# MathisWellmann/gym-rs

Measured on AMD Instinct MI355X. Metric: env-steps/sec (whole node), CartPole-v1 @ 2^20 envs per MI355X, higher is better.
Workload: dtype f32

## Files before the change

### gym-rs_amd/csrc/gymrs_philox.h

```cpp
#pragma once
#include "gymrs_math.h"

namespace gymrs {

struct u32x4 {
    uint32_t v[4];
};

constexpr uint32_t kPhiloxM0 = 0xD2511F53u, kPhiloxM1 = 0xCD9E8D57u;
constexpr uint32_t kPhiloxW0 = 0x9E3779B9u, kPhiloxW1 = 0xBB67AE85u;

GYMRS_HD uint32_t xor3(uint32_t a, uint32_t b, uint32_t c)
{
#if defined(__HIP_DEVICE_COMPILE__)
    return __builtin_amdgcn_bitop3_b32(a, b, c, 0x96);
#else
    return a ^ b ^ c;
#endif
}

GYMRS_HD u32x4 philox4x32_10(uint32_t c0, uint32_t c1, uint32_t c2, uint32_t c3, uint32_t k0, uint32_t k1)
{
#if defined(__HIPCC__)
#pragma unroll
#endif
    for (int round = 0; round < 10; ++round) {
        uint64_t p0 = (uint64_t)kPhiloxM0 * c0;
        uint64_t p1 = (uint64_t)kPhiloxM1 * c2;
        uint32_t n0 = xor3((uint32_t)(p1 >> 32), c1, k0);
        uint32_t n2 = xor3((uint32_t)(p0 >> 32), c3, k1);
        c1 = (uint32_t)p1;
        c3 = (uint32_t)p0;
        c0 = n0;
        c2 = n2;
        k0 += kPhiloxW0;
        k1 += kPhiloxW1;
    }
    return u32x4{{c0, c1, c2, c3}};
}

constexpr uint32_t kStreamReset = 0, kStreamAction = 1;

GYMRS_HD u32x4 draw4(uint64_t seed, uint64_t gid, uint64_t tick, uint32_t stream)
{
    return philox4x32_10((uint32_t)gid, (uint32_t)(gid >> 32), (uint32_t)tick,
                         ((uint32_t)(tick >> 32) & 0xffffu) | (stream << 16), (uint32_t)seed,
                         (uint32_t)(seed >> 32));
}

GYMRS_HD u32x4 action_block(uint64_t seed, uint64_t gid, uint64_t slot) { return draw4(seed, gid >> 2, slot, kStreamAction); }
GYMRS_HD uint32_t pick_word(const u32x4& b, uint32_t j) { return j == 0 ? b.v[0] : (j == 1 ? b.v[1] : (j == 2 ? b.v[2] : b.v[3])); }
GYMRS_HD uint32_t action_word(uint64_t seed, uint64_t gid, uint64_t t) { return pick_word(action_block(seed, gid, t), (uint32_t)gid & 3u); }
GYMRS_HD uint8_t discrete_from_word(uint32_t word, uint64_t t, uint32_t n_actions)
{
    const uint32_t half = (word >> (((uint32_t)t & 1u) * 16u)) & 0xffffu;
    return (uint8_t)((half * n_actions) >> 16);
}
GYMRS_HD uint8_t action_discrete(uint64_t seed, uint64_t gid, uint64_t t, uint32_t n_actions)
{
    return discrete_from_word(action_word(seed, gid, t >> 1), t, n_actions);
}

struct SampleBox {
    float lo[4], scale24[4], hi_prev[4];
};

inline SampleBox make_sample_box(const float* lo, const float* hi, int dims)
{
    SampleBox b;
    for (int j = 0; j < 4; ++j) {
        b.lo[j] = 0.0f;
        b.scale24[j] = 0.0f;
        b.hi_prev[j] = 0.0f;
    }
    for (int j = 0; j < dims; ++j) {
        b.lo[j] = lo[j];
        b.scale24[j] = (hi[j] - lo[j]) * 0x1p-24f;
        uint32_t h = f2u(hi[j]);
        h = (hi[j] > 0.0f) ? h - 1u : ((h & 0x7fffffffu) == 0u ? 0x80000001u : h + 1u);
        b.hi_prev[j] = u2f(h);
    }
    return b;
}

GYMRS_HD float uniform_in_box(uint32_t r, const SampleBox& b, int j)
{
    const float v = fmaf_((float)(r >> 8), b.scale24[j], b.lo[j]);
    return v < b.hi_prev[j] ? v : b.hi_prev[j];
}

GYMRS_HD float uniform_between(uint32_t r, float low, float high)
{
    SampleBox b;
    b.lo[0] = low;
    b.scale24[0] = (high - low) * 0x1p-24f;
    uint32_t h = f2u(high);
    h = (high > 0.0f) ? h - 1u : ((h & 0x7fffffffu) == 0u ? 0x80000001u : h + 1u);
    b.hi_prev[0] = u2f(h);
    return uniform_in_box(r, b, 0);
}

}
```

### gym-rs_amd/csrc/gymrs_step_impl.h

```cpp
#pragma once
#include "gymrs_tile.h"

namespace gymrs {

__device__ __forceinline__ uint32_t select_by_mask(unsigned long long m, uint32_t fresh, uint32_t ep)
{
    uint32_t r;
    asm("v_cndmask_b32_e64 %0, %1, %2, %3" : "=v"(r) : "v"(ep), "v"(fresh), "s"(m));
    return r;
}

template <class Env, int VEC, uint32_t FLAGS, int THREADS, bool FULL>
__device__ __forceinline__ void step_block_loaded(StepArgs a, const typename Env::Consts& c, ResetLds<Env, VEC, THREADS>& lds, uint32_t vblock,
                                                  TileRegs<Env, VEC, FLAGS>& d)
{
    constexpr int kVec = VEC;
    constexpr int LPB = THREADS * kVec;
    constexpr bool AUTO = (FLAGS & GYMRS_AUTO_RESET) != 0;
    constexpr bool STATS = AUTO && (FLAGS & GYMRS_TRACK_STATS);
    constexpr bool LOGGED = TileRegs<Env, VEC, FLAGS>::LOGGED;
    const uint64_t base = (uint64_t)vblock * LPB + (uint64_t)threadIdx.x * kVec;
    if (a.tick_base) a.tick += *a.tick_base;
    unsigned long long old_resets = 0;
    double old_ret = 0.0, open = 0.0;
    const size_t wave_slot = (size_t)vblock * (THREADS / 64) + (threadIdx.x >> 6);
    if (STATS && !LOGGED) {
        const unsigned long long* bs = a.block_stats + wave_slot * 2;
        old_resets = bs[0];
        if (!Env::kConstReward) {
            old_ret = reinterpret_cast<const double*>(bs)[1];
            open = a.wave_open[wave_slot];
        }
    }
    constexpr int kOlder = (int)kResetLogRows - 1;
    Vec<uint32_t, VEC> ep;
    unsigned long long older = 0;
    [[maybe_unused]] unsigned long long* older_at = nullptr;
    const bool fold = LOGGED && a.fold_step != 0;
    if (fold) {
        ep = load_vec<uint32_t, kVec, false>(a.ep_start, base, a.n, FULL, 0u);
        const uint32_t lane = threadIdx.x & 63u;
        older_at = a.reset_log + (size_t)((uint32_t)(a.tick - 1 - (uint64_t)(lane / kVec)) & (kResetLogRows - 1u)) * a.reset_log_row_words +
                   wave_slot * kVec + lane % kVec;
        if (lane < (uint32_t)(kOlder * kVec)) older = *older_at;
        old_resets = a.block_stats[wave_slot * 2];
    }
    constexpr bool CAN_ELIDE = AUTO && Env::kConstReward;
    const bool elide = CAN_ELIDE && (Env::kElideConstReward || a.elide_reward != 0u);
    uint32_t clean = 0;
    if (elide) clean = a.wave_clean[wave_slot];
#ifndef GYMRS_EXP_XCC_PARTS
#define GYMRS_EXP_XCC_PARTS 7
#endif
    uint32_t xcc_want = 0, xcc_id = 0;
    const bool xcc_asks = a.xcc_check != 0u && (uint32_t)__builtin_amdgcn_readfirstlane((int)threadIdx.x) < 64u && vblock == blockIdx.x * (uint32_t)kStepTiles;
#if GYMRS_EXP_XCC_PARTS & 1
    if (xcc_asks && a.xcc_check == 1u) xcc_want = a.xcc_table[(blockIdx.x & 7u) * kXccTableStride];
#endif
#if GYMRS_EXP_XCC_PARTS & 2
    if (xcc_asks) {
        asm volatile("s_getreg_b32 %0, hwreg(HW_REG_XCC_ID)" : "=s"(xcc_id));
        xcc_id = (a.xcc_seq << 8) | ((xcc_id & 0xfu) + 1u);
    }
#endif
    GYMRS_STAMP(1);
    StepOut<VEC> out;
    advance_tile<Env, VEC, FLAGS, FULL, false, THREADS>(a, c, base, d, lds, old_resets, old_ret, open, out, vblock);
    store_tile<Env, VEC, FLAGS, FULL>(a, base, d, out, elide && clean != 0 && out.reward_is_const);
    if (fold) {
        const uint32_t lane = threadIdx.x & 63u;
        uint32_t finished = wave_sum_u32((uint32_t)__popcll(older));
#pragma unroll
        for (int k = 0; k < kVec; ++k) finished += (uint32_t)__popcll(out.masks[k]);
        if (finished != 0) {
#pragma unroll
            for (int s = kOlder - 1; s >= 0; --s) {
                const uint32_t fresh = (uint32_t)(a.tick - (uint64_t)s);
#pragma unroll
                for (int k = 0; k < kVec; ++k) {
                    const unsigned long long m = ((unsigned long long)(uint32_t)__builtin_amdgcn_readlane((int)(uint32_t)(older >> 32), s * kVec + k) << 32) |
                                                 (uint32_t)__builtin_amdgcn_readlane((int)(uint32_t)older, s * kVec + k);
                    ep.v[k] = select_by_mask(m, fresh, ep.v[k]);
                }
            }
            const uint32_t fresh_now = (uint32_t)(a.tick + 1);
#pragma unroll
            for (int k = 0; k < kVec; ++k) ep.v[k] = select_by_mask(out.masks[k], fresh_now, ep.v[k]);
            store_vec<uint32_t, kVec, false>(a.ep_start, base, a.n, FULL, ep);
            if (older != 0) *older_at = 0;
            if (lane == 0) a.block_stats[wave_slot * 2] = old_resets + finished;
        }
    }
    if (elide && (clean != 0) != out.reward_is_const && (threadIdx.x & 63u) == 0) a.wave_clean[wave_slot] = out.reward_is_const ? 1u : 0u;
    if (STATS && !Env::kConstReward && (threadIdx.x & 63u) == 0) a.wave_open[wave_slot] = open;
#if GYMRS_EXP_XCC_PARTS & 4
    if (xcc_asks) {
        if (a.xcc_check == 2u) {
            if (blockIdx.x < 8u && threadIdx.x == 0) a.xcc_table[blockIdx.x * kXccTableStride] = xcc_id;
        } else if (xcc_want != xcc_id && threadIdx.x == 0) {
            a.err_seen[1] = blockIdx.x + 1u;
        }
    }
#endif
    GYMRS_STAMP(6);
}

template <class Env, int VEC, uint32_t FLAGS, int THREADS, bool FULL>
__device__ __forceinline__ void step_block(const StepArgs& a, const typename Env::Consts& c, ResetLds<Env, VEC, THREADS>& lds, uint32_t vblock)
{
    GYMRS_STAMP(0);
    TileRegs<Env, VEC, FLAGS> d;
    load_tile<Env, VEC, FLAGS, FULL>(a, (uint64_t)vblock * (THREADS * VEC) + (uint64_t)threadIdx.x * VEC, d);
    load_param_index<Env, VEC, FLAGS, FULL>(a, c, (uint64_t)vblock * (THREADS * VEC) + (uint64_t)threadIdx.x * VEC, d);
    step_block_loaded<Env, VEC, FLAGS, THREADS, FULL>(a, c, lds, vblock, d);
}

template <class Env>
struct KernArgView {
    using Consts = typename Env::Consts;
    static __device__ __forceinline__ void fetch(StepArgs& a, Consts& c)
    {
        const char* kp = (const char*)__builtin_amdgcn_kernarg_segment_ptr();
        __builtin_memcpy(&a, kp + offsetof(StepKernArgs<Consts>, rest), sizeof(StepArgs));
        __builtin_memcpy(&c, kp + offsetof(StepKernArgs<Consts>, c), sizeof(Consts));
    }
};

template <class Env, int VEC, uint32_t FLAGS, int THREADS>
__device__ __forceinline__ void step_kernel_body(float* s0, float* s1, float* s2, float* s3, const void* action, uint64_t n_fast, const StepArgs& rest,
                                                 const typename Env::Consts& c_by_value)
{
    constexpr int LPB = THREADS * VEC;
    __shared__ ResetLds<Env, VEC, THREADS> lds;
    if constexpr (kStepTiles == 1 && Env::kLoadsAheadOfArguments) {
        StepArgs a;
        typename Env::Consts c;
        if ((uint64_t)blockIdx.x * LPB + (uint64_t)((threadIdx.x >> 6) + 1) * (64 * VEC) <= n_fast) {
#ifdef GYMRS_TRACE_TIMES
            const unsigned long long t_start = __builtin_amdgcn_s_memtime();
#endif
            using R = TileRegs<Env, VEC, FLAGS>;
            using Action = typename Env::Action;
            const uint64_t base = (uint64_t)blockIdx.x * LPB + (uint64_t)threadIdx.x * VEC;
            float* const sp[4] = {s0, s1, s2, s3};
            TileRegs<Env, VEC, FLAGS> d;
#pragma unroll
            for (int j = 0; j < Env::kState; ++j) d.st[j] = load_vec<float, VEC, R::NT_SL>(sp[j], base, n_fast, true, 0.0f);
            d.act = load_vec<Action, VEC, R::NT_A>(static_cast<const Action*>(action), base, n_fast, true, Action(0));
            __builtin_amdgcn_sched_barrier(0);
            KernArgView<Env>::fetch(a, c);
            a.s[0] = s0;
            a.s[1] = s1;
            a.s[2] = s2;
            a.s[3] = s3;
            a.action = action;
#ifdef GYMRS_TRACE_TIMES
            if (a.trace && (threadIdx.x & 63u) == 0) a.trace[((size_t)blockIdx.x * a.trace_wpb + (threadIdx.x >> 6)) * 8 + 0] = t_start;
#endif
            if (Env::kHasBeyond && !R::AUTO) d.beyond = load_vec<uint8_t, VEC, R::NT_SL>(a.beyond, base, a.n, true, uint8_t(0));
            if (R::TLIM && !Env::kNeverTerminates) d.ep_start = load_vec<uint32_t, VEC, false>(a.ep_start, base, a.n, true, 0u);
            load_param_index<Env, VEC, FLAGS, true>(a, c, base, d);
            step_block_loaded<Env, VEC, FLAGS, THREADS, true>(a, c, lds, blockIdx.x, d);
        } else {
            KernArgView<Env>::fetch(a, c);
            a.s[0] = s0;
            a.s[1] = s1;
            a.s[2] = s2;
            a.s[3] = s3;
            a.action = action;
            step_block<Env, VEC, FLAGS, THREADS, false>(a, c, lds, blockIdx.x);
        }
    } else {
        const typename Env::Consts& c = c_by_value;
        StepArgs a = rest;
        a.s[0] = s0;
        a.s[1] = s1;
        a.s[2] = s2;
        a.s[3] = s3;
        a.action = action;
        if constexpr (kStepTiles == 1) {
            if ((uint64_t)blockIdx.x * LPB + (uint64_t)((threadIdx.x >> 6) + 1) * (64 * VEC) <= n_fast)
                step_block<Env, VEC, FLAGS, THREADS, true>(a, c, lds, blockIdx.x);
            else
                step_block<Env, VEC, FLAGS, THREADS, false>(a, c, lds, blockIdx.x);
        } else {
            const uint32_t vb0 = blockIdx.x * (uint32_t)kStepTiles;
            if ((uint64_t)(vb0 + kStepTiles - 1) * LPB + (uint64_t)((threadIdx.x >> 6) + 1) * (64 * VEC) <= n_fast) {
                TileRegs<Env, VEC, FLAGS> d[2];
                load_tile<Env, VEC, FLAGS, true>(a, (uint64_t)vb0 * LPB + (uint64_t)threadIdx.x * VEC, d[0]);
                load_param_index<Env, VEC, FLAGS, true>(a, c, (uint64_t)vb0 * LPB + (uint64_t)threadIdx.x * VEC, d[0]);
#pragma unroll
                for (int j = 0; j < kStepTiles; ++j) {
                    if (j + 1 < kStepTiles) {
                        load_tile<Env, VEC, FLAGS, true>(a, (uint64_t)(vb0 + j + 1) * LPB + (uint64_t)threadIdx.x * VEC, d[(j + 1) & 1]);
                        load_param_index<Env, VEC, FLAGS, true>(a, c, (uint64_t)(vb0 + j + 1) * LPB + (uint64_t)threadIdx.x * VEC, d[(j + 1) & 1]);
                    }
                    step_block_loaded<Env, VEC, FLAGS, THREADS, true>(a, c, lds, vb0 + j, d[j & 1]);
                }
            } else {
                for (int j = 0; j < kStepTiles; ++j)
                    if ((uint64_t)(vb0 + j) * LPB < rest.n) step_block<Env, VEC, FLAGS, THREADS, false>(a, c, lds, vb0 + j);
            }
        }
    }
}

#ifndef GYMRS_EXP_WAVES
#define GYMRS_EXP_WAVES(VEC_) (16 / (VEC_) < 1 ? 1 : 16 / (VEC_))
#endif
#ifndef GYMRS_EXP_WAVES_MIN
#define GYMRS_EXP_WAVES_MIN 1
#endif
#define GYMRS_STEP_KERNEL_ATTRS(THREADS_, VEC_) \
    __global__ __launch_bounds__(THREADS_) __attribute__((amdgpu_waves_per_eu(GYMRS_EXP_WAVES_MIN, GYMRS_EXP_WAVES(VEC_))))

template <class Env, int VEC, uint32_t FLAGS, int THREADS>
GYMRS_STEP_KERNEL_ATTRS(THREADS, VEC) void step_kernel(float* s0, float* s1, float* s2, float* s3, const void* action, uint64_t n_fast,
                                                       const StepArgs rest, const typename Env::Consts c)
{
    step_kernel_body<Env, VEC, FLAGS, THREADS>(s0, s1, s2, s3, action, n_fast, rest, c);
}

#ifndef GYMRS_EXP_BLOCK
static_assert(CartPoleT::kThreads == kCartPoleThreads && MountainCarT::kThreads == kBlock && PendulumT::kThreads == kBlock,
              "step_threads_of (gymrs_kernels.h) must pick what launch_one picks");
#endif

template <class Env, int VEC, uint32_t FLAGS>
static hipError_t launch_one(const StepArgs& a, const void* consts, hipStream_t stream)
{
    launch_begin();
    if constexpr (Env::kThreads != kBlock) {
        if (step_uses_big_groups(a.n, Env::kThreads, VEC)) {
            hipLaunchKernelGGL((step_kernel<Env, VEC, FLAGS, Env::kThreads>), dim3(step_grid(a.n, VEC, Env::kThreads * kStepTiles)), dim3(Env::kThreads), 0,
                               stream, a.s[0], a.s[1], a.s[2], a.s[3], a.action, a.n_fast, a, *static_cast<const typename Env::Consts*>(consts));
            return hipGetLastError();
        }
    }
    hipLaunchKernelGGL((step_kernel<Env, VEC, FLAGS, kBlock>), dim3(step_grid(a.n, VEC, kBlock * kStepTiles)), dim3(kBlock), 0, stream, a.s[0], a.s[1],
                       a.s[2], a.s[3], a.action, a.n_fast, a, *static_cast<const typename Env::Consts*>(consts));
    return hipGetLastError();
}

template <class Env, int VEC, uint32_t NTBIT>
static hipError_t launch_flags_nt(uint32_t flags, const StepArgs& a, const void* consts, hipStream_t stream)
{
    constexpr uint32_t A = GYMRS_AUTO_RESET, S = GYMRS_TRACK_STATS, T = GYMRS_TIME_LIMIT, F = GYMRS_FINAL_OBS;
    if (!(flags & A)) flags &= ~(S | F);
    switch (flags & (A | S | T | F)) {
#ifdef GYMRS_DEV_MINIMAL
    case A | S: return launch_one<Env, VEC, A | S | NTBIT>(a, consts, stream);
    case A | S | T: return launch_one<Env, VEC, A | S | T | NTBIT>(a, consts, stream);
    default: return hipErrorInvalidValue;
#else
    case 0: return launch_one<Env, VEC, 0 | NTBIT>(a, consts, stream);
    case A: return launch_one<Env, VEC, A | NTBIT>(a, consts, stream);
    case A | S: return launch_one<Env, VEC, A | S | NTBIT>(a, consts, stream);
    case T: return launch_one<Env, VEC, T | NTBIT>(a, consts, stream);
    case A | T: return launch_one<Env, VEC, A | T | NTBIT>(a, consts, stream);
    case A | S | T: return launch_one<Env, VEC, A | S | T | NTBIT>(a, consts, stream);
    case A | F: return launch_one<Env, VEC, A | F | NTBIT>(a, consts, stream);
    case A | S | F: return launch_one<Env, VEC, A | S | F | NTBIT>(a, consts, stream);
    case A | T | F: return launch_one<Env, VEC, A | T | F | NTBIT>(a, consts, stream);
    case A | S | T | F: return launch_one<Env, VEC, A | S | T | F | NTBIT>(a, consts, stream);
    default: return hipErrorInvalidValue;
#endif
    }
}

template <class Env, int VEC>
static hipError_t launch_flags(uint32_t flags, const StepArgs& a, const void* consts, hipStream_t stream)
{
    if (flags & kFlagNonTemporal) return launch_flags_nt<Env, VEC, kFlagNonTemporal>(flags, a, consts, stream);
    if (flags & kFlagNtOut) return launch_flags_nt<Env, VEC, kFlagNtOut>(flags, a, consts, stream);
    return launch_flags_nt<Env, VEC, 0u>(flags, a, consts, stream);
}

template <class Env>
static hipError_t launch_vec(int vec, uint32_t flags, const StepArgs& a, const void* consts, hipStream_t stream)
{
    switch (vec) {
    case 4: return launch_flags<Env, 4>(flags, a, consts, stream);
#ifndef GYMRS_DEV_MINIMAL
    case 8: return launch_flags<Env, 8>(flags, a, consts, stream);
#endif
    default: return hipErrorInvalidValue;
    }
}

}
```

### gym-rs_amd/csrc/gymrs_tile.h

```cpp
#pragma once
#include <type_traits>

#include "gymrs_kernels.h"

namespace gymrs {


#ifdef GYMRS_TRACE_TIMES
#define GYMRS_STAMP(slot_)                                                                                   \
    do {                                                                                                     \
        if (a.trace && (threadIdx.x & 63u) == 0)                                                             \
            a.trace[((size_t)blockIdx.x * a.trace_wpb + (threadIdx.x >> 6)) * 8 + (slot_)] = __builtin_amdgcn_s_memtime(); \
    } while (0)
#else
#define GYMRS_STAMP(slot_) do { } while (0)
#endif

__device__ __forceinline__ float wave_sum(float v)
{
    auto dpp_add = [](float x, auto ctrl, auto row_mask) {
        const int moved = __builtin_amdgcn_update_dpp(0, __builtin_bit_cast(int, x), decltype(ctrl)::value, decltype(row_mask)::value, 0xf, true);
        return x + __builtin_bit_cast(float, moved);
    };
    using std::integral_constant;
    v = dpp_add(v, integral_constant<int, 0xb1>{}, integral_constant<int, 0xf>{});
    v = dpp_add(v, integral_constant<int, 0x4e>{}, integral_constant<int, 0xf>{});
    v = dpp_add(v, integral_constant<int, 0x141>{}, integral_constant<int, 0xf>{});
    v = dpp_add(v, integral_constant<int, 0x140>{}, integral_constant<int, 0xf>{});
    v = dpp_add(v, integral_constant<int, 0x142>{}, integral_constant<int, 0xa>{});
    v = dpp_add(v, integral_constant<int, 0x143>{}, integral_constant<int, 0xc>{});
    return __builtin_bit_cast(float, __builtin_amdgcn_readlane(__builtin_bit_cast(int, v), 63));
}

__device__ __forceinline__ uint32_t wave_sum_u32(uint32_t v)
{
    auto dpp_add = [](uint32_t x, auto ctrl, auto row_mask) {
        return x + (uint32_t)__builtin_amdgcn_update_dpp(0, (int)x, decltype(ctrl)::value, decltype(row_mask)::value, 0xf, true);
    };
    using std::integral_constant;
    v = dpp_add(v, integral_constant<int, 0xb1>{}, integral_constant<int, 0xf>{});
    v = dpp_add(v, integral_constant<int, 0x4e>{}, integral_constant<int, 0xf>{});
    v = dpp_add(v, integral_constant<int, 0x141>{}, integral_constant<int, 0xf>{});
    v = dpp_add(v, integral_constant<int, 0x140>{}, integral_constant<int, 0xf>{});
    v = dpp_add(v, integral_constant<int, 0x142>{}, integral_constant<int, 0xa>{});
    v = dpp_add(v, integral_constant<int, 0x143>{}, integral_constant<int, 0xc>{});
    return (uint32_t)__builtin_amdgcn_readlane((int)v, 63);
}

template <class T, int V>
struct alignas(sizeof(T) * V) Vec {
    T v[V];
};

template <class T, int V, bool NT>
__device__ __forceinline__ Vec<T, V> load_vec(const T* __restrict__ p, uint64_t base, uint64_t n, bool full, T fill)
{
    typedef T vt __attribute__((ext_vector_type(V)));
    Vec<T, V> r;
    if (full) {
        const vt x = NT ? __builtin_nontemporal_load(reinterpret_cast<const vt*>(p + base)) : *reinterpret_cast<const vt*>(p + base);
#pragma unroll
        for (int k = 0; k < V; ++k) r.v[k] = x[k];
    } else {
#pragma unroll
        for (int k = 0; k < V; ++k) r.v[k] = (base + k < n) ? p[base + k] : fill;
    }
    return r;
}

template <class T, int V, int POL>
__device__ __forceinline__ void store_vec(T* __restrict__ p, uint64_t base, uint64_t n, bool full, const Vec<T, V>& r)
{
    typedef T vt __attribute__((ext_vector_type(V)));
    if (full) {
        vt x;
#pragma unroll
        for (int k = 0; k < V; ++k) x[k] = r.v[k];
        if constexpr (POL == 2) {
            static_assert(sizeof(vt) == 4 || sizeof(vt) == 16, "sc1 stores: 4 lanes per work-item only");
            if constexpr (sizeof(vt) == 16) {
                typedef uint32_t u4 __attribute__((ext_vector_type(4)));
                asm volatile("global_store_dwordx4 %0, %1, off sc1\n\ts_nop 1" ::"v"(reinterpret_cast<vt*>(p + base)), "v"(__builtin_bit_cast(u4, x)) : "memory");
            }
            else
                asm volatile("global_store_dword %0, %1, off sc1\n\ts_nop 1" ::"v"(reinterpret_cast<vt*>(p + base)), "v"(__builtin_bit_cast(uint32_t, x)) : "memory");
        } else if constexpr (POL == 1)
            __builtin_nontemporal_store(x, reinterpret_cast<vt*>(p + base));
        else
            *reinterpret_cast<vt*>(p + base) = x;
    } else {
#pragma unroll
        for (int k = 0; k < V; ++k)
            if (base + k < n) p[base + k] = r.v[k];
    }
}

template <int VEC>
__device__ __forceinline__ void obs_sincos(const Vec<float, VEC>& theta, Vec<float, VEC>& oc, Vec<float, VEC>& os)
{
    bool med = true;
#pragma unroll
    for (int k = 0; k < VEC; ++k) med = med && in_short_range(theta.v[k]);
    if (__all(med)) {
#pragma unroll
        for (int k = 0; k < VEC; ++k) sincos_short(theta.v[k], &os.v[k], &oc.v[k]);
    } else {
#pragma unroll
        for (int k = 0; k < VEC; ++k) sincosf_(theta.v[k], &os.v[k], &oc.v[k]);
    }
}

struct CartPoleT {
    using Consts = CartPoleConsts;
    static constexpr bool kTable = false;
    using Action = uint8_t;
    static constexpr int kState = 4;
    static constexpr int kSampled = 4;
    static constexpr bool kConstReward = true;
    static constexpr float kReward = 1.0f;
    static constexpr bool kElideConstReward = false;
#ifdef GYMRS_EXP_NO_RESET_LOG
    static constexpr bool kUseResetLog = false;
#else
    static constexpr bool kUseResetLog = true;
#endif
    static constexpr bool kHasBeyond = true;
    static constexpr bool kHasObsExtra = false;
    static constexpr bool kNeverTerminates = false;
    static constexpr int kThreads = 512;
    static constexpr bool kLoadsAheadOfArguments = true;
    __device__ static bool valid(Action a) { return a < 2; }
    __device__ static void advance(const Consts& c, float* st, Action a, float& reward, bool& done)
    {
        done = cartpole_advance(c, st[0], st[1], st[2], st[3], a);
        reward = 1.0f;
    }
    static constexpr uint32_t kActions = 2;
    static constexpr uint32_t kRangeMax = 0x3f490fdbu;
    __device__ static uint32_t range_key(const float* st) { return f2u(st[2]) & 0x7fffffffu; }
    static constexpr int kVariants = 2;
    __device__ static int variant(const Consts& c) { return c.integrator == 0 ? 0 : 1; }
    template <int INTEG>
    __device__ static void advance_fast(const Consts& c, float* st, Action a, float& reward, bool& done)
    {
        done = cartpole_advance<SinCosSmall, INTEG>(c, st[0], st[1], st[2], st[3], a);
        reward = 1.0f;
    }
    __device__ static void sample(const u32x4& r, const SampleBox& b, float* st) { cartpole_sample(r, b, st[0], st[1], st[2], st[3]); }
};

struct MountainCarT {
    using Consts = MountainCarConsts;
    static constexpr bool kTable = false;
    using Action = uint8_t;
    static constexpr int kState = 2;
    static constexpr int kSampled = 1;
    static constexpr bool kConstReward = true;
    static constexpr float kReward = -1.0f;
    static constexpr bool kElideConstReward = true;
    static constexpr bool kUseResetLog = false;
    static constexpr bool kHasBeyond = false;
    static constexpr bool kHasObsExtra = false;
    static constexpr bool kNeverTerminates = false;
    static constexpr int kThreads = 256;
    static constexpr bool kLoadsAheadOfArguments = false;
    __device__ static bool valid(Action a) { return a < 3; }
    __device__ static void advance(const Consts& c, float* st, Action a, float& reward, bool& done)
    {
        done = mountain_car_advance(c, st[0], st[1], a);
        reward = -1.0f;
    }
    static constexpr uint32_t kActions = 3;
    static constexpr uint32_t kRangeMax = 0x43480000u;
    __device__ static uint32_t range_key(const float* st) { return f2u(3.0f * st[0]) & 0x7fffffffu; }
    static constexpr int kVariants = 1;
    __device__ static int variant(const Consts&) { return 0; }
    template <int>
    __device__ static void advance_fast(const Consts& c, float* st, Action a, float& reward, bool& done)
    {
        done = mountain_car_advance<SinCosShort>(c, st[0], st[1], a);
        reward = -1.0f;
    }
    __device__ static void sample(const u32x4& r, const SampleBox& b, float* st) { mountain_car_sample(r, b, st[0], st[1]); }
};

struct PendulumT {
    using Consts = PendulumConsts;
    static constexpr bool kTable = false;
    using Action = float;
    static constexpr int kState = 2;
    static constexpr int kSampled = 2;
    static constexpr bool kConstReward = false;
    static constexpr float kReward = 0.0f;
    static constexpr bool kElideConstReward = false;
    static constexpr bool kUseResetLog = false;
    static constexpr bool kHasBeyond = false;
    static constexpr bool kHasObsExtra = true;
    static constexpr bool kNeverTerminates = true;
    static constexpr int kThreads = 256;
    static constexpr bool kLoadsAheadOfArguments = true;
    __device__ static bool valid(Action) { return true; }
    __device__ static void advance(const Consts& c, float* st, Action a, float& reward, bool& done)
    {
        reward = pendulum_advance(c, st[0], st[1], a);
        done = false;
    }
    static constexpr uint32_t kActions = 0;
    static constexpr uint32_t kRangeMax = 0x43480000u;
    __device__ static uint32_t range_key(const float* st) { return f2u(st[0]) & 0x7fffffffu; }
    static constexpr int kVariants = 1;
    __device__ static int variant(const Consts&) { return 0; }
    template <int>
    __device__ static void advance_fast(const Consts& c, float* st, Action a, float& reward, bool& done)
    {
        reward = pendulum_advance<SinCosShort>(c, st[0], st[1], a);
        done = false;
    }
    __device__ static void sample(const u32x4& r, const SampleBox& b, float* st) { pendulum_sample(r, b, st[0], st[1]); }
};

template <class Base>
struct TableT : Base {
    static_assert(!Base::kNeverTerminates, "no Pendulum tables: max_torque also drives the random-policy actions");
    static constexpr bool kTable = true;
    using LaneConsts = typename Base::Consts;
    using Consts = TableConsts;
    __device__ static int variant(const Consts& c) { return Base::kVariants == 1 || c.integrator == 0 ? 0 : 1; }
    __device__ static LaneConsts lane_consts(const Consts& c, const ParamRow& r)
    {
        LaneConsts l;
        consts_of_row(r, c.integrator, c.max_steps, l);
        return l;
    }
};

template <class Env, class = void>
struct TableLane {
    struct type {};
};
template <class Env>
struct TableLane<Env, std::enable_if_t<Env::kTable>> {
    using type = typename Env::LaneConsts;
};

template <class Env, int VEC, uint32_t FLAGS>
struct TileRegs {
    static constexpr bool AUTO = (FLAGS & GYMRS_AUTO_RESET) != 0;
    static constexpr bool STATS = AUTO && (FLAGS & GYMRS_TRACK_STATS) != 0;
    static constexpr bool TLIM = (FLAGS & GYMRS_TIME_LIMIT) != 0;
    static constexpr bool FINAL = AUTO && (FLAGS & GYMRS_FINAL_OBS) != 0;
    static_assert(!FINAL || !(Env::kHasBeyond && !AUTO), "StepArgs::final_obs shares the slot of `beyond`: no FINAL kernel may read beyond");
    static constexpr bool NT = (FLAGS & kFlagNonTemporal) != 0;
#ifdef GYMRS_EXP_HINTS
    static constexpr bool NT_SL = (GYMRS_EXP_HINTS & 1) != 0, NT_SS = (GYMRS_EXP_HINTS & 2) != 0, NT_A = (GYMRS_EXP_HINTS & 4) != 0,
                          NT_O = (GYMRS_EXP_HINTS & 8) != 0;
#else
    static constexpr bool NT_SL = NT || (FLAGS & kFlagNtStateLoads) != 0, NT_SS = NT, NT_A = NT, NT_O = NT || (FLAGS & kFlagNtOut) != 0;
#endif
#ifdef GYMRS_EXP_SC1
    static constexpr int POL_SS = (VEC == 4 && (GYMRS_EXP_SC1 & 2)) ? 2 : (NT_SS ? 1 : 0), POL_O = (VEC == 4 && (GYMRS_EXP_SC1 & 8)) ? 2 : (NT_O ? 1 : 0);
#else
    static constexpr int POL_SS = NT_SS ? 1 : 0, POL_O = NT_O ? 1 : 0;
#endif
    static constexpr bool LOGGED = STATS && !TLIM && Env::kConstReward && Env::kUseResetLog;
    Vec<float, VEC> st[Env::kState];
    Vec<typename Env::Action, VEC> act;
    Vec<uint8_t, VEC> beyond;
    Vec<uint32_t, VEC> ep_start;
    Vec<uint16_t, VEC> pidx;
};

template <class Env, int VEC, uint32_t FLAGS, bool FULL>
__device__ __forceinline__ void load_param_index(const StepArgs& a, const typename Env::Consts& c, uint64_t base, TileRegs<Env, VEC, FLAGS>& d)
{
    if constexpr (Env::kTable) d.pidx = load_vec<uint16_t, VEC, false>(c.index, base, a.n, FULL, uint16_t(0));
}

template <class Env, int VEC, uint32_t FLAGS, bool FULL, bool ROLL = false>
__device__ __forceinline__ void load_tile(const StepArgs& a, uint64_t base, TileRegs<Env, VEC, FLAGS>& d)
{
    constexpr int kVec = VEC;
    using R = TileRegs<Env, VEC, FLAGS>;
    using Action = typename Env::Action;
#pragma unroll
    for (int j = 0; j < Env::kState; ++j) d.st[j] = load_vec<float, kVec, R::NT_SL>(a.s[j], base, a.n, FULL, 0.0f);
    if (!ROLL) d.act = load_vec<Action, kVec, R::NT_A>(static_cast<const Action*>(a.action), base, a.n, FULL, Action(0));
    if (Env::kHasBeyond && !R::AUTO) d.beyond = load_vec<uint8_t, kVec, R::NT_SL>(a.beyond, base, a.n, FULL, uint8_t(0));
    if (ROLL ? (R::STATS || R::TLIM) : (R::TLIM && !Env::kNeverTerminates))
        d.ep_start = load_vec<uint32_t, kVec, false>(a.ep_start, base, a.n, FULL, 0u);
}

template <class Env, int VEC, int THREADS = Env::kThreads>
struct ResetLds {
    static constexpr int kLanes = THREADS * VEC;
    uint16_t list[kLanes];
    struct alignas(Env::kState * 4) State {
        float v[Env::kState];
    };
    State fresh[kLanes];
};

template <class Env, int VEC, int V>
__device__ __forceinline__ void advance_fast_all(const typename Env::Consts& c, float (&ls)[Env::kState][VEC],
                                                 const typename Env::Action (&la)[VEC], float (&rw)[VEC], bool (&dn)[VEC])
{
    constexpr int kVec = VEC;
    constexpr int NS = Env::kState;
#pragma unroll
    for (int k = 0; k < kVec; ++k) {
        float lane_st[NS];
#pragma unroll
        for (int j = 0; j < NS; ++j) lane_st[j] = ls[j][k];
        Env::template advance_fast<V>(c, lane_st, la[k], rw[k], dn[k]);
#pragma unroll
        for (int j = 0; j < NS; ++j) ls[j][k] = lane_st[j];
    }
}

template <class Env, int VEC, int V>
__device__ __forceinline__ void advance_fast_rows(const typename Env::LaneConsts (&lc)[VEC], float (&ls)[Env::kState][VEC],
                                                  const typename Env::Action (&la)[VEC], float (&rw)[VEC], bool (&dn)[VEC])
{
    constexpr int NS = Env::kState;
#pragma unroll
    for (int k = 0; k < VEC; ++k) {
        float lane_st[NS];
#pragma unroll
        for (int j = 0; j < NS; ++j) lane_st[j] = ls[j][k];
        Env::template advance_fast<V>(lc[k], lane_st, la[k], rw[k], dn[k]);
#pragma unroll
        for (int j = 0; j < NS; ++j) ls[j][k] = lane_st[j];
    }
}

template <class Env, int VEC, uint32_t FLAGS>
__device__ __forceinline__ bool lane_index_ok(const typename Env::Consts& c, const TileRegs<Env, VEC, FLAGS>& d, int k)
{
    if constexpr (Env::kTable)
        return d.pidx.v[k] < c.k;
    else
        return true;
}

template <uint32_t N, class A, int VEC>
__device__ __forceinline__ bool actions_all_below(const Vec<A, VEC>& act)
{
    if constexpr (N == 0 || sizeof(A) != 1) {
        return true;
    } else {
        static_assert(N == 2 || N == 3, "only Discrete(2) and Discrete(3) are packed here");
        struct Words {
            uint32_t w[VEC / 4];
        };
        const Words words = __builtin_bit_cast(Words, act);
        uint32_t bad = 0;
#pragma unroll
        for (int i = 0; i < VEC / 4; ++i) {
            const uint32_t x = words.w[i];
            bad |= N == 2 ? (x & 0xfefefefeu) : ((x & 0xfcfcfcfcu) | (x & (x >> 1) & 0x01010101u));
        }
        return bad == 0;
    }
}

template <int VEC>
struct StepOut {
    Vec<float, VEC> reward;
    Vec<uint8_t, VEC> done, trunc;
    bool reward_is_const;
    unsigned long long masks[VEC];
};

template <class Env, int VEC, uint32_t FLAGS, bool FULL>
__device__ __forceinline__ void store_final_obs(const StepArgs& a, uint64_t base, const float (&ls)[Env::kState][VEC], const bool (&need_reset)[VEC])
{
    using R = TileRegs<Env, VEC, FLAGS>;
    static_assert(R::FINAL, "final-observation stores belong to GYMRS_FINAL_OBS instantiations only");
    const uint64_t stride = final_obs_stride(a.n);
    float* const fo = a.final_obs;
    if constexpr (Env::kHasObsExtra) {
        static_assert(Env::kNeverTerminates && Env::kState == 2, "the obs_extra env is Pendulum: (cos, sin, theta_dot), one shared episode clock");
        Vec<float, VEC> th, td, oc, os;
#pragma unroll
        for (int k = 0; k < VEC; ++k) {
            th.v[k] = ls[0][k];
            td.v[k] = ls[1][k];
        }
        obs_sincos<VEC>(th, oc, os);
        if (FULL) {
            store_vec<float, VEC, R::POL_O>(fo, base, a.n, true, oc);
            store_vec<float, VEC, R::POL_O>(fo + stride, base, a.n, true, os);
            store_vec<float, VEC, R::POL_O>(fo + 2 * stride, base, a.n, true, td);
        } else {
#pragma unroll
            for (int k = 0; k < VEC; ++k) {
                if (need_reset[k]) {
                    fo[base + k] = oc.v[k];
                    fo[stride + base + k] = os.v[k];
                    fo[2 * stride + base + k] = td.v[k];
                }
            }
        }
    } else {
#pragma unroll
        for (int k = 0; k < VEC; ++k) {
            if (need_reset[k]) {
#pragma unroll
                for (int j = 0; j < Env::kState; ++j) fo[(uint64_t)j * stride + base + k] = ls[j][k];
            }
        }
    }
}

template <class Env, int VEC, uint32_t FLAGS, bool FULL, bool ROLL = false, int THREADS = Env::kThreads>
__device__ __forceinline__ void advance_tile(const StepArgs& a, const typename Env::Consts& c, uint64_t base,
                                             TileRegs<Env, VEC, FLAGS>& d, ResetLds<Env, VEC, THREADS>& lds, unsigned long long& resets,
                                             double& ret, double& open, StepOut<VEC>& out, uint32_t vblock)
{
    static_assert(Env::kConstReward || Env::kNeverTerminates,
                  "return tracking assumes a constant reward (return = +-length) or one shared episode clock");
    constexpr int kVec = VEC;
    using R = TileRegs<Env, VEC, FLAGS>;
    constexpr bool AUTO = R::AUTO, STATS = R::STATS, TLIM = R::TLIM;
    constexpr bool LOGGED = R::LOGGED && !ROLL;
    constexpr int NS = Env::kState;
    using Action = typename Env::Action;
    const uint32_t tick_next = (uint32_t)(a.tick + 1);

    float ls[NS][kVec];
    Action la[kVec];
#pragma unroll
    for (int k = 0; k < kVec; ++k) {
        la[k] = d.act.v[k];
#pragma unroll
        for (int j = 0; j < NS; ++j) ls[j][k] = d.st[j].v[k];
    }
    float rw[kVec];
    bool dn[kVec], tr[kVec], need_reset[kVec];
#ifdef GYMRS_TRACE_TIMES
    asm volatile("s_waitcnt vmcnt(0)" ::: "memory");
    GYMRS_STAMP(2);
#endif
    uint32_t key = 0;
#pragma unroll
    for (int k = 0; k < kVec; ++k) {
        float lane_st[NS];
#pragma unroll
        for (int j = 0; j < NS; ++j) lane_st[j] = ls[j][k];
        const uint32_t kk = Env::range_key(lane_st);
        key = key > kk ? key : kk;
    }
    bool fast = FULL && key <= Env::kRangeMax && actions_all_below<Env::kActions>(d.act);
    [[maybe_unused]] typename TableLane<Env>::type lc[kVec];
    if constexpr (Env::kTable) {
        uint32_t top = 0;
#pragma unroll
        for (int k = 0; k < kVec; ++k) {
            uint32_t i = d.pidx.v[k];
            if (ROLL) asm volatile("" : "+v"(i));
            top = top > i ? top : i;
            lc[k] = Env::lane_consts(c, c.rows[i < c.k ? i : 0u]);
        }
        fast = fast && top < c.k;
    }
    out.reward_is_const = true;
#pragma unroll
    for (int k = 0; k < kVec; ++k) out.masks[k] = 0;
    if (__all(fast)) {
        if constexpr (Env::kTable) {
            if (Env::kVariants == 1 || Env::variant(c) == 0)
                advance_fast_rows<Env, VEC, 0>(lc, ls, la, rw, dn);
            else
                advance_fast_rows<Env, VEC, 1>(lc, ls, la, rw, dn);
        } else {
            if (Env::kVariants == 1 || Env::variant(c) == 0)
                advance_fast_all<Env, VEC, 0>(c, ls, la, rw, dn);
            else
                advance_fast_all<Env, VEC, 1>(c, ls, la, rw, dn);
        }
    } else {
        uint32_t n_bad = 0, first_bad = 0xffffffffu;
#pragma unroll
        for (int k = 0; k < kVec; ++k) {
            const bool live = FULL || (base + k < a.n);
            const bool ok = Env::valid(la[k]) && lane_index_ok(c, d, k);
            float lane_st[NS];
#pragma unroll
            for (int j = 0; j < NS; ++j) lane_st[j] = ls[j][k];
            float r = 0.0f;
            bool dk = false;
            if (live && ok) {
                if constexpr (Env::kTable)
                    Env::advance(lc[k], lane_st, la[k], r, dk);
                else
                    Env::advance(c, lane_st, la[k], r, dk);
            } else if (live) {
                n_bad += 1;
                first_bad = min(first_bad, (uint32_t)(base + k));
            }
#pragma unroll
            for (int j = 0; j < NS; ++j) ls[j][k] = lane_st[j];
            rw[k] = r;
            dn[k] = dk;
        }
        if (n_bad) {
            atomicAdd(&a.err[0], n_bad);
            atomicMin(&a.err[1], first_bad);
            *a.err_seen = 1u;
        }
        out.reward_is_const = __all(n_bad == 0);
    }
    GYMRS_STAMP(3);
    Vec<uint8_t, kVec>&done = out.done, &trunc = out.trunc;
#pragma unroll
    for (int k = 0; k < kVec; ++k) {
        const bool stepped = (FULL || (base + k < a.n)) && Env::valid(la[k]) && lane_index_ok(c, d, k);
        if (Env::kHasBeyond && !AUTO) {
            bool b = d.beyond.v[k] != 0;
            const float r = cartpole_reward(dn[k], b);
            if (stepped) {
                rw[k] = r;
                d.beyond.v[k] = b ? 1 : 0;
            }
        }
        if (Env::kNeverTerminates)
            tr[k] = TLIM && stepped && a.truncate_all != 0;
        else
            tr[k] = TLIM && stepped && (tick_next - d.ep_start.v[k]) >= c.max_steps;
        done.v[k] = dn[k] ? 1 : 0;
        trunc.v[k] = tr[k] ? 1 : 0;
        need_reset[k] = AUTO && (dn[k] || tr[k]);
    }
    if (STATS && !Env::kConstReward) {
        float rs = 0.0f;
#pragma unroll
        for (int k = 0; k < kVec; ++k) rs += rw[k];
        open += (double)wave_sum(rs);
    }

#ifdef GYMRS_EXP_EARLY_OUT
    if (!ROLL && !Env::kElideConstReward) {
#pragma unroll
        for (int k = 0; k < kVec; ++k) out.reward.v[k] = rw[k];
        store_vec<float, kVec, R::POL_O>(a.reward, base, a.n, FULL, out.reward);
        if (!Env::kNeverTerminates) store_vec<uint8_t, kVec, R::POL_O>(a.done, base, a.n, FULL, out.done);
        if (TLIM && !(Env::kNeverTerminates && a.skip_trunc_store)) store_vec<uint8_t, kVec, R::POL_O>(a.truncated, base, a.n, FULL, out.trunc);
    }
#endif
    if (AUTO) {
        constexpr int LPW = 64 * kVec;
        const uint32_t tid = threadIdx.x, wave = tid >> 6, lane = tid & 63u;
        uint16_t* list = lds.list + wave * LPW;
        uint32_t slot[kVec];
        uint32_t total = 0;
#pragma unroll
        for (int k = 0; k < kVec; ++k) {
            const unsigned long long m = __ballot(need_reset[k]);
            out.masks[k] = m;
            const uint32_t rank = __builtin_amdgcn_mbcnt_hi((uint32_t)(m >> 32), __builtin_amdgcn_mbcnt_lo((uint32_t)m, 0u));
            slot[k] = total + rank;
            if (need_reset[k]) {
                list[slot[k]] = (uint16_t)(lane * kVec + k);
            }
            total += (uint32_t)__popcll(m);
        }
        if (total != 0) {
            if constexpr (R::FINAL) store_final_obs<Env, VEC, FLAGS, FULL>(a, base, ls, need_reset);
            if (LOGGED && a.fold_step == 0 && lane == 0) {
                typedef unsigned long long ull2 __attribute__((ext_vector_type(2)));
                const size_t wave_slot = (size_t)vblock * (THREADS / 64) + wave;
                ull2* row = reinterpret_cast<ull2*>(a.reset_log + (size_t)((uint32_t)a.tick & (kResetLogRows - 1u)) * a.reset_log_row_words +
                                                    wave_slot * kVec);
#pragma unroll
                for (int k = 0; k < kVec; k += 2) row[k / 2] = ull2{out.masks[k], out.masks[k + 1]};
            }
            __builtin_amdgcn_fence(__ATOMIC_RELEASE, "wavefront");
            __builtin_amdgcn_wave_barrier();
            const uint64_t wave_base = base - (uint64_t)lane * kVec;
            for (uint32_t i = lane; i < total; i += 64u) {
                const uint64_t gl = wave_base + list[i];
                const u32x4 r = draw4(a.seed, a.gid0 + gl, a.tick, kStreamReset);
                float ns[NS];
                Env::sample(r, a.box, ns);
                typename ResetLds<Env, VEC, THREADS>::State fs;
#pragma unroll
                for (int j = 0; j < NS; ++j) fs.v[j] = ns[j];
                lds.fresh[wave * LPW + i] = fs;
                if (!ROLL && !LOGGED && (STATS || TLIM)) a.ep_start[gl] = tick_next;
            }
            __builtin_amdgcn_fence(__ATOMIC_RELEASE, "wavefront");
            __builtin_amdgcn_wave_barrier();
#pragma unroll
            for (int k = 0; k < kVec; ++k) {
                if (need_reset[k]) {
                    const typename ResetLds<Env, VEC, THREADS>::State fs = lds.fresh[wave * LPW + slot[k]];
#pragma unroll
                    for (int j = 0; j < NS; ++j) ls[j][k] = fs.v[j];
                    if (ROLL && (STATS || TLIM)) d.ep_start.v[k] = tick_next;
                }
            }
            if (STATS && !LOGGED) {
                unsigned long long* bs = a.block_stats + ((size_t)vblock * (THREADS / 64) + wave) * 2;
                if (!Env::kConstReward) {
                    ret += open;
                    open = 0.0;
                    if (!ROLL && lane == 0) reinterpret_cast<double*>(bs)[1] = ret;
                }
                resets += total;
                if (!ROLL && lane == 0) bs[0] = resets;
            }
        }
    }
    GYMRS_STAMP(4);
#pragma unroll
    for (int k = 0; k < kVec; ++k) {
        out.reward.v[k] = rw[k];
#pragma unroll
        for (int j = 0; j < NS; ++j) d.st[j].v[k] = ls[j][k];
    }
}

template <class Env, int VEC, uint32_t FLAGS, bool FULL, bool ROLL = false>
__device__ __forceinline__ void store_tile(const StepArgs& a, uint64_t base, const TileRegs<Env, VEC, FLAGS>& d,
                                           const StepOut<VEC>& out, bool skip_reward = false)
{
    constexpr int kVec = VEC;
    using R = TileRegs<Env, VEC, FLAGS>;
    constexpr bool AUTO = R::AUTO, STATS = R::STATS, TLIM = R::TLIM;
#pragma unroll
    for (int j = 0; j < Env::kState; ++j) store_vec<float, kVec, R::POL_SS>(a.s[j], base, a.n, FULL, d.st[j]);
#ifdef GYMRS_EXP_EARLY_OUT
    constexpr bool kOutStored = !ROLL && !Env::kElideConstReward;
#else
    constexpr bool kOutStored = false;
#endif
    if (!skip_reward && !kOutStored) store_vec<float, kVec, R::POL_O>(a.reward, base, a.n, FULL, out.reward);
    if (!Env::kNeverTerminates && !kOutStored) store_vec<uint8_t, kVec, R::POL_O>(a.done, base, a.n, FULL, out.done);
    if (TLIM && !kOutStored && !(Env::kNeverTerminates && a.skip_trunc_store)) store_vec<uint8_t, kVec, R::POL_O>(a.truncated, base, a.n, FULL, out.trunc);
    if (Env::kHasBeyond && !AUTO) store_vec<uint8_t, kVec, R::POL_SS>(a.beyond, base, a.n, FULL, d.beyond);
    if (ROLL && (STATS || TLIM)) store_vec<uint32_t, kVec, 0>(a.ep_start, base, a.n, FULL, d.ep_start);
    if (Env::kHasObsExtra) {
        Vec<float, kVec> oc, os;
        bool med = true;
#pragma unroll
        for (int k = 0; k < kVec; ++k) med = med && in_short_range(d.st[0].v[k]);
        if (__all(med)) {
#pragma unroll
            for (int k = 0; k < kVec; ++k) sincos_short(d.st[0].v[k], &os.v[k], &oc.v[k]);
        } else {
#pragma unroll
            for (int k = 0; k < kVec; ++k) sincosf_(d.st[0].v[k], &os.v[k], &oc.v[k]);
        }
        store_vec<float, kVec, R::POL_O>(a.obs_cos, base, a.n, FULL, oc);
        store_vec<float, kVec, R::POL_O>(a.obs_sin, base, a.n, FULL, os);
    }
    GYMRS_STAMP(5);
#ifdef GYMRS_TRACE_TIMES
    asm volatile("s_waitcnt vmcnt(0)" ::: "memory");
#endif
}


}
```

Baseline: 154.5 billion.

## Precompute reset Philox keys and LDS addresses under loads for CartPole

For CartPole only, a RearmSetup object is built before advance_tile. It precomputes the Philox key schedule, the tick-dependent first-round product, LDS list/fresh byte offsets and the reset-log row, pinned in VGPRs so this work can hide under outstanding loads. The reset path then uses a Philox variant that skips the key additions and the first-round M1 multiply. The tick_base and xcc_table loads become scalar-constant loads, with the tick folded in late. This raises VGPR pressure and adds complexity to reduce the latency of the per-step reset path.

```diff
diff --git a/gym-rs_amd/csrc/gymrs_philox.h b/gym-rs_amd/csrc/gymrs_philox.h
--- a/gym-rs_amd/csrc/gymrs_philox.h
+++ b/gym-rs_amd/csrc/gymrs_philox.h
@@ -35,6 +35,48 @@
         c2 = n2;
         k0 += kPhiloxW0;
         k1 += kPhiloxW1;
+    }
+    return u32x4{{c0, c1, c2, c3}};
+}
+
+struct PhiloxKeys {
+    uint32_t k0[10], k1[10];
+};
+
+GYMRS_HD PhiloxKeys philox_key_schedule(uint32_t k0, uint32_t k1)
+{
+    PhiloxKeys ks;
+#if defined(__HIPCC__)
+#pragma unroll
+#endif
+    for (int round = 0; round < 10; ++round) {
+        ks.k0[round] = k0;
+        ks.k1[round] = k1;
+        k0 += kPhiloxW0;
+        k1 += kPhiloxW1;
+    }
+    return ks;
+}
+
+GYMRS_HD u32x4 philox4x32_10_prepared(uint32_t c0, uint32_t c1, uint32_t c3, uint32_t p1_hi, uint32_t p1_lo, const PhiloxKeys& ks)
+{
+    const uint64_t q0 = (uint64_t)kPhiloxM0 * c0;
+    uint32_t c2 = xor3((uint32_t)(q0 >> 32), c3, ks.k1[0]);
+    c0 = xor3(p1_hi, c1, ks.k0[0]);
+    c1 = p1_lo;
+    c3 = (uint32_t)q0;
+#if defined(__HIPCC__)
+#pragma unroll
+#endif
+    for (int round = 1; round < 10; ++round) {
+        uint64_t p0 = (uint64_t)kPhiloxM0 * c0;
+        uint64_t p1 = (uint64_t)kPhiloxM1 * c2;
+        uint32_t n0 = xor3((uint32_t)(p1 >> 32), c1, ks.k0[round]);
+        uint32_t n2 = xor3((uint32_t)(p0 >> 32), c3, ks.k1[round]);
+        c1 = (uint32_t)p1;
+        c3 = (uint32_t)p0;
+        c0 = n0;
+        c2 = n2;
     }
     return u32x4{{c0, c1, c2, c3}};
 }
diff --git a/gym-rs_amd/csrc/gymrs_step_impl.h b/gym-rs_amd/csrc/gymrs_step_impl.h
--- a/gym-rs_amd/csrc/gymrs_step_impl.h
+++ b/gym-rs_amd/csrc/gymrs_step_impl.h
@@ -20,7 +20,17 @@
     constexpr bool STATS = AUTO && (FLAGS & GYMRS_TRACK_STATS);
     constexpr bool LOGGED = TileRegs<Env, VEC, FLAGS>::LOGGED;
     const uint64_t base = (uint64_t)vblock * LPB + (uint64_t)threadIdx.x * kVec;
-    if (a.tick_base) a.tick += *a.tick_base;
+    constexpr bool SETUP = Env::kSetupUnderLoads && AUTO;
+    [[maybe_unused]] uint64_t tick_add = 0;
+    [[maybe_unused]] bool tick_late = false;
+    if constexpr (SETUP) {
+        if (a.tick_base) {
+            tick_add = load_uniform_invariant(a.tick_base);
+            tick_late = true;
+        }
+    } else {
+        if (a.tick_base) a.tick += *a.tick_base;
+    }
     unsigned long long old_resets = 0;
     double old_ret = 0.0, open = 0.0;
     const size_t wave_slot = (size_t)vblock * (THREADS / 64) + (threadIdx.x >> 6);
@@ -38,6 +48,10 @@
     [[maybe_unused]] unsigned long long* older_at = nullptr;
     const bool fold = LOGGED && a.fold_step != 0;
     if (fold) {
+        if constexpr (SETUP) {
+            a.tick += tick_add;
+            tick_late = false;
+        }
         ep = load_vec<uint32_t, kVec, false>(a.ep_start, base, a.n, FULL, 0u);
         const uint32_t lane = threadIdx.x & 63u;
         older_at = a.reset_log + (size_t)((uint32_t)(a.tick - 1 - (uint64_t)(lane / kVec)) & (kResetLogRows - 1u)) * a.reset_log_row_words +
@@ -55,7 +69,12 @@
     uint32_t xcc_want = 0, xcc_id = 0;
     const bool xcc_asks = a.xcc_check != 0u && (uint32_t)__builtin_amdgcn_readfirstlane((int)threadIdx.x) < 64u && vblock == blockIdx.x * (uint32_t)kStepTiles;
 #if GYMRS_EXP_XCC_PARTS & 1
-    if (xcc_asks && a.xcc_check == 1u) xcc_want = a.xcc_table[(blockIdx.x & 7u) * kXccTableStride];
+    if (xcc_asks && a.xcc_check == 1u) {
+        if constexpr (SETUP)
+            xcc_want = load_uniform_invariant(a.xcc_table + (blockIdx.x & 7u) * kXccTableStride);
+        else
+            xcc_want = a.xcc_table[(blockIdx.x & 7u) * kXccTableStride];
+    }
 #endif
 #if GYMRS_EXP_XCC_PARTS & 2
     if (xcc_asks) {
@@ -65,7 +84,16 @@
 #endif
     GYMRS_STAMP(1);
     StepOut<VEC> out;
-    advance_tile<Env, VEC, FLAGS, FULL, false, THREADS>(a, c, base, d, lds, old_resets, old_ret, open, out, vblock);
+    if constexpr (SETUP) {
+        RearmSetup<Env, VEC, THREADS> pre(a, vblock);
+        pre.tick_late = tick_late;
+        pre.tick_add = tick_add;
+        __builtin_amdgcn_sched_barrier(0);
+        advance_tile<Env, VEC, FLAGS, FULL, false, THREADS, RearmSetup<Env, VEC, THREADS>>(a, c, base, d, lds, old_resets, old_ret, open, out, vblock, pre);
+        if (elide) asm volatile("" : "+v"(clean));
+    } else {
+        advance_tile<Env, VEC, FLAGS, FULL, false, THREADS>(a, c, base, d, lds, old_resets, old_ret, open, out, vblock);
+    }
     store_tile<Env, VEC, FLAGS, FULL>(a, base, d, out, elide && clean != 0 && out.reward_is_const);
     if (fold) {
         const uint32_t lane = threadIdx.x & 63u;
@@ -149,6 +177,11 @@
             d.act = load_vec<Action, VEC, R::NT_A>(static_cast<const Action*>(action), base, n_fast, true, Action(0));
             __builtin_amdgcn_sched_barrier(0);
             KernArgView<Env>::fetch(a, c);
+            if constexpr (Env::kSetupUnderLoads && R::AUTO) {
+                asm volatile("" ::"s"(a.reward), "s"(a.done), "s"(a.err), "s"(a.err_seen), "s"(a.xcc_table), "s"(a.xcc_check), "s"(a.xcc_seq), "s"(c.integrator));
+                if constexpr (R::TLIM) asm volatile("" ::"s"(a.truncated), "s"(c.max_steps));
+                if constexpr (R::FINAL) asm volatile("" ::"s"(a.final_obs));
+            }
             a.s[0] = s0;
             a.s[1] = s1;
             a.s[2] = s2;
diff --git a/gym-rs_amd/csrc/gymrs_tile.h b/gym-rs_amd/csrc/gymrs_tile.h
--- a/gym-rs_amd/csrc/gymrs_tile.h
+++ b/gym-rs_amd/csrc/gymrs_tile.h
@@ -129,6 +129,7 @@
     static constexpr bool kNeverTerminates = false;
     static constexpr int kThreads = 512;
     static constexpr bool kLoadsAheadOfArguments = true;
+    static constexpr bool kSetupUnderLoads = true;
     __device__ static bool valid(Action a) { return a < 2; }
     __device__ static void advance(const Consts& c, float* st, Action a, float& reward, bool& done)
     {
@@ -164,6 +165,7 @@
     static constexpr bool kNeverTerminates = false;
     static constexpr int kThreads = 256;
     static constexpr bool kLoadsAheadOfArguments = false;
+    static constexpr bool kSetupUnderLoads = false;
     __device__ static bool valid(Action a) { return a < 3; }
     __device__ static void advance(const Consts& c, float* st, Action a, float& reward, bool& done)
     {
@@ -199,6 +201,7 @@
     static constexpr bool kNeverTerminates = true;
     static constexpr int kThreads = 256;
     static constexpr bool kLoadsAheadOfArguments = true;
+    static constexpr bool kSetupUnderLoads = false;
     __device__ static bool valid(Action) { return true; }
     __device__ static void advance(const Consts& c, float* st, Action a, float& reward, bool& done)
     {
@@ -223,6 +226,7 @@
 struct TableT : Base {
     static_assert(!Base::kNeverTerminates, "no Pendulum tables: max_torque also drives the random-policy actions");
     static constexpr bool kTable = true;
+    static constexpr bool kSetupUnderLoads = false;
     using LaneConsts = typename Base::Consts;
     using Consts = TableConsts;
     __device__ static int variant(const Consts& c) { return Base::kVariants == 1 || c.integrator == 0 ? 0 : 1; }
@@ -300,6 +304,72 @@
     State fresh[kLanes];
 };
 
+__device__ __forceinline__ void keep_in_vgpr(uint32_t& x) { asm volatile("" : "+v"(x)); }
+__device__ __forceinline__ void keep_in_vgpr(float& x) { asm volatile("" : "+v"(x)); }
+
+template <class T>
+__device__ __forceinline__ T load_uniform_invariant(const T* p)
+{
+    return *(const __attribute__((address_space(4))) T*)p;
+}
+
+struct NoRearmSetup {};
+
+template <class Env, int VEC, int THREADS>
+struct RearmSetup {
+    using Lds = ResetLds<Env, VEC, THREADS>;
+    static constexpr uint32_t kLanesPerWave = 64u * VEC;
+    PhiloxKeys keys;
+    SampleBox box;
+    uint32_t lane;
+    uint32_t lane_first;
+    uint32_t list_mine;
+    uint32_t fresh_mine;
+    uint32_t wave;
+    uint64_t wave_base;
+    uint32_t p1_hi, p1_lo, c3;
+    uint64_t log_row;
+    bool tick_late = false;
+    uint64_t tick_add = 0;
+
+    __device__ __forceinline__ void retick(const StepArgs& a, uint64_t tick, uint32_t vblock)
+    {
+        const uint64_t p1 = (uint64_t)kPhiloxM1 * (uint32_t)tick;
+        p1_hi = (uint32_t)(p1 >> 32);
+        p1_lo = (uint32_t)p1;
+        c3 = ((uint32_t)(tick >> 32) & 0xffffu) | (kStreamReset << 16);
+        const size_t wave_slot = (size_t)vblock * (THREADS / 64) + wave;
+        log_row = (uint64_t)(a.reset_log + (size_t)((uint32_t)tick & (kResetLogRows - 1u)) * a.reset_log_row_words + wave_slot * VEC);
+    }
+
+    __device__ __forceinline__ RearmSetup(const StepArgs& a, uint32_t vblock)
+    {
+        lane = threadIdx.x & 63u;
+        wave = (uint32_t)__builtin_amdgcn_readfirstlane((int)(threadIdx.x >> 6));
+        lane_first = lane * VEC;
+        list_mine = (uint32_t)offsetof(Lds, list) + (wave * kLanesPerWave + lane) * (uint32_t)sizeof(uint16_t);
+        fresh_mine = (uint32_t)offsetof(Lds, fresh) + (wave * kLanesPerWave + lane) * (uint32_t)sizeof(typename Lds::State);
+        wave_base = (uint64_t)vblock * (THREADS * VEC) + (uint64_t)wave * kLanesPerWave;
+        keys = philox_key_schedule((uint32_t)a.seed, (uint32_t)(a.seed >> 32));
+        box = a.box;
+        keep_in_vgpr(lane);
+        keep_in_vgpr(lane_first);
+        keep_in_vgpr(list_mine);
+        keep_in_vgpr(fresh_mine);
+        keep_in_vgpr(keys.k0[0]);
+        keep_in_vgpr(keys.k1[0]);
+        keep_in_vgpr(keys.k0[1]);
+#pragma unroll
+        for (int j = 0; j < Env::kSampled; ++j) {
+            keep_in_vgpr(box.lo[j]);
+            keep_in_vgpr(box.hi_prev[j]);
+        }
+        retick(a, a.tick, vblock);
+    }
+    __device__ __forceinline__ uint32_t list_wave() const { return (uint32_t)offsetof(Lds, list) + wave * kLanesPerWave * (uint32_t)sizeof(uint16_t); }
+    __device__ __forceinline__ uint32_t fresh_wave() const { return (uint32_t)offsetof(Lds, fresh) + wave * kLanesPerWave * (uint32_t)sizeof(typename Lds::State); }
+};
+
 template <class Env, int VEC, int V>
 __device__ __forceinline__ void advance_fast_all(const typename Env::Consts& c, float (&ls)[Env::kState][VEC],
                                                  const typename Env::Action (&la)[VEC], float (&rw)[VEC], bool (&dn)[VEC])
@@ -412,11 +482,13 @@
     }
 }
 
-template <class Env, int VEC, uint32_t FLAGS, bool FULL, bool ROLL = false, int THREADS = Env::kThreads>
+template <class Env, int VEC, uint32_t FLAGS, bool FULL, bool ROLL = false, int THREADS = Env::kThreads, class Setup = NoRearmSetup>
 __device__ __forceinline__ void advance_tile(const StepArgs& a, const typename Env::Consts& c, uint64_t base,
                                              TileRegs<Env, VEC, FLAGS>& d, ResetLds<Env, VEC, THREADS>& lds, unsigned long long& resets,
-                                             double& ret, double& open, StepOut<VEC>& out, uint32_t vblock)
-{
+                                             double& ret, double& open, StepOut<VEC>& out, uint32_t vblock, Setup pre = Setup{})
+{
+    constexpr bool PRE = !std::is_same_v<Setup, NoRearmSetup>;
+    static_assert(!PRE || !ROLL, "the rollout kernel's tick changes inside the kernel: nothing to prepare once");
     static_assert(Env::kConstReward || Env::kNeverTerminates,
                   "return tracking assumes a constant reward (return = +-length) or one shared episode clock");
     constexpr int kVec = VEC;
@@ -425,7 +497,8 @@
     constexpr bool LOGGED = R::LOGGED && !ROLL;
     constexpr int NS = Env::kState;
     using Action = typename Env::Action;
-    const uint32_t tick_next = (uint32_t)(a.tick + 1);
+    uint64_t tick = a.tick;
+    uint32_t tick_next = (uint32_t)(a.tick + 1);
 
     float ls[NS][kVec];
     Action la[kVec];
@@ -511,6 +584,13 @@
         out.reward_is_const = __all(n_bad == 0);
     }
     GYMRS_STAMP(3);
+    if constexpr (PRE) {
+        if (pre.tick_late) {
+            tick += pre.tick_add;
+            tick_next = (uint32_t)(tick + 1);
+            pre.retick(a, tick, vblock);
+        }
+    }
     Vec<uint8_t, kVec>&done = out.done, &trunc = out.trunc;
 #pragma unroll
     for (int k = 0; k < kVec; ++k) {
@@ -549,8 +629,11 @@
 #endif
     if (AUTO) {
         constexpr int LPW = 64 * kVec;
-        const uint32_t tid = threadIdx.x, wave = tid >> 6, lane = tid & 63u;
+        const uint32_t tid = threadIdx.x, wave = tid >> 6;
+        uint32_t lane = tid & 63u;
+        if constexpr (PRE) lane = pre.lane;
         uint16_t* list = lds.list + wave * LPW;
+        [[maybe_unused]] char* const lds_bytes = reinterpret_cast<char*>(&lds);
         uint32_t slot[kVec];
         uint32_t total = 0;
 #pragma unroll
@@ -560,7 +643,10 @@
             const uint32_t rank = __builtin_amdgcn_mbcnt_hi((uint32_t)(m >> 32), __builtin_amdgcn_mbcnt_lo((uint32_t)m, 0u));
             slot[k] = total + rank;
             if (need_reset[k]) {
-                list[slot[k]] = (uint16_t)(lane * kVec + k);
+                if constexpr (PRE)
+                    *reinterpret_cast<uint16_t*>(lds_bytes + (pre.list_wave() + slot[k] * (uint32_t)sizeof(uint16_t))) = (uint16_t)(pre.lane_first + k);
+                else
+                    list[slot[k]] = (uint16_t)(lane * kVec + k);
             }
             total += (uint32_t)__popcll(m);
         }
@@ -569,13 +655,34 @@
             if (LOGGED && a.fold_step == 0 && lane == 0) {
                 typedef unsigned long long ull2 __attribute__((ext_vector_type(2)));
                 const size_t wave_slot = (size_t)vblock * (THREADS / 64) + wave;
-                ull2* row = reinterpret_cast<ull2*>(a.reset_log + (size_t)((uint32_t)a.tick & (kResetLogRows - 1u)) * a.reset_log_row_words +
-                                                    wave_slot * kVec);
+                ull2* row;
+                if constexpr (PRE)
+                    row = reinterpret_cast<ull2*>(pre.log_row);
+                else
+                    row = reinterpret_cast<ull2*>(a.reset_log + (size_t)((uint32_t)a.tick & (kResetLogRows - 1u)) * a.reset_log_row_words +
+                                                  wave_slot * kVec);
 #pragma unroll
                 for (int k = 0; k < kVec; k += 2) row[k / 2] = ull2{out.masks[k], out.masks[k + 1]};
             }
             __builtin_amdgcn_fence(__ATOMIC_RELEASE, "wavefront");
             __builtin_amdgcn_wave_barrier();
+            if constexpr (PRE) {
+                const uint64_t gid_wave = a.gid0 + pre.wave_base;
+                uint32_t list_at = pre.list_mine, fresh_at = pre.fresh_mine;
+                for (uint32_t i = lane; i < total; i += 64u, list_at += 64u * (uint32_t)sizeof(uint16_t),
+                              fresh_at += 64u * (uint32_t)sizeof(typename ResetLds<Env, VEC, THREADS>::State)) {
+                    const uint32_t wl = *reinterpret_cast<const uint16_t*>(lds_bytes + list_at);
+                    const uint64_t gid = gid_wave + wl;
+                    const u32x4 r = philox4x32_10_prepared((uint32_t)gid, (uint32_t)(gid >> 32), pre.c3, pre.p1_hi, pre.p1_lo, pre.keys);
+                    float ns[NS];
+                    Env::sample(r, pre.box, ns);
+                    typename ResetLds<Env, VEC, THREADS>::State fs;
+#pragma unroll
+                    for (int j = 0; j < NS; ++j) fs.v[j] = ns[j];
+                    *reinterpret_cast<typename ResetLds<Env, VEC, THREADS>::State*>(lds_bytes + fresh_at) = fs;
+                    if (!LOGGED && (STATS || TLIM)) a.ep_start[pre.wave_base + wl] = tick_next;
+                }
+            } else {
             const uint64_t wave_base = base - (uint64_t)lane * kVec;
             for (uint32_t i = lane; i < total; i += 64u) {
                 const uint64_t gl = wave_base + list[i];
@@ -588,12 +695,18 @@
                 lds.fresh[wave * LPW + i] = fs;
                 if (!ROLL && !LOGGED && (STATS || TLIM)) a.ep_start[gl] = tick_next;
             }
+            }
             __builtin_amdgcn_fence(__ATOMIC_RELEASE, "wavefront");
             __builtin_amdgcn_wave_barrier();
 #pragma unroll
             for (int k = 0; k < kVec; ++k) {
                 if (need_reset[k]) {
-                    const typename ResetLds<Env, VEC, THREADS>::State fs = lds.fresh[wave * LPW + slot[k]];
+                    typename ResetLds<Env, VEC, THREADS>::State fs;
+                    if constexpr (PRE)
+                        fs = *reinterpret_cast<const typename ResetLds<Env, VEC, THREADS>::State*>(
+                            lds_bytes + (pre.fresh_wave() + slot[k] * (uint32_t)sizeof(typename ResetLds<Env, VEC, THREADS>::State)));
+                    else
+                        fs = lds.fresh[wave * LPW + slot[k]];
 #pragma unroll
                     for (int j = 0; j < NS; ++j) ls[j][k] = fs.v[j];
                     if (ROLL && (STATS || TLIM)) d.ep_start.v[k] = tick_next;
```

Measured after the change: 158.2 billion (median of 3 runs). Within noise of the previous version (+2.4%).
